# FraPria/proovread

Hardware: AMD Instinct MI355X
Metric: corrected long-read Mbases/sec per node (higher is better)
Workload: dtype int32

## Files before the change

### proovread_amd/csrc/seed.cpp

```cpp
#include <algorithm>
#include <atomic>
#include <cstdlib>
#include <cstring>
#include <string>
#include <thread>
#include <utility>
#include <vector>

#include <sys/mman.h>

#include "../../include/prgpu.h"
#include "err.h"
#include "seed_core.h"
#include "seed_dev.h"

namespace seedc = prgpu::seedc;

namespace {

constexpr int KI = 12;
constexpr uint32_t NK = 1u << (2 * KI);
constexpr uint8_t SEP = 5;
constexpr int KX = 28;
constexpr uint64_t KX_MASK = (1ull << (2 * KX)) - 1;

template <class T>
struct BigAlloc {
    using value_type = T;
    static constexpr size_t kHuge = (size_t)32 << 20;
    BigAlloc() = default;
    template <class U>
    BigAlloc(const BigAlloc<U> &) {}
    T *allocate(size_t n) {
        const size_t bytes = n * sizeof(T);
        if (bytes >= kHuge) {
// ... 620 lines not shown
        uint64_t v = 0;
        for (int k = 0; k < 16; ++k) {
            const int64_t x = (int64_t)w * 16 + k;
            v |= (uint64_t)(x < V.n_text ? V.text[x] : SEP) << (4 * k);
        }
        text4[w] = v;
    }
    return text4;
}

extern "C" int pr_seed_map_device_caps(const pr_seed_index *h, const pr_seed_opts *o, const uint8_t *sr_seq,
                                       const int64_t *sr_off, int n_sr, int n_threads, pr_seed_tasks *out,
                                       int32_t *status) {
    if (!h || !o || !out || !status || n_sr < 0 || (n_sr && (!sr_seq || !sr_off)))
        return pr_set_error(PR_ERR_ARG, "null arg");
    if (o->min_seed_len < KI) return pr_set_error(PR_ERR_UNSUPPORTED, "min seed length below the 12-mer index");
    out->n = 0;
    out->t = nullptr;
    seedc::IndexView V = view_of(h->I);
    int qmax = 1;
    for (int i = 0; i < n_sr; ++i) qmax = std::max<int>(qmax, (int)(sr_off[i + 1] - sr_off[i]));
    const std::vector<uint64_t> text4 = pack_text4(V);
    V.text4 = text4.data();
    seedc::Caps caps = seedc::device_caps(qmax);
    caps.hi = V.ksplit != nullptr;
    caps.lazy = seedc::lazy_occ(*o) ? 1 : 0;
    const int64_t bytes = seedc::scratch_bytes(caps);
    int nt = n_threads > 0 ? n_threads : (int)std::thread::hardware_concurrency();
    nt = nt < 1 ? 1 : (nt > 64 ? 64 : nt);
    std::vector<ReadOut> res(n_sr);
    std::atomic<int> next{0};
    const char *fe = getenv("PRGPU_SCRATCH_FILL");
    const uint64_t fill = fe ? 0x0101010101010101ull * (uint64_t)(strtoul(fe, nullptr, 0) & 0xFF) : 0;
    auto work = [&]() {
        std::vector<uint64_t> slab((size_t)(bytes / 8 + 1), fill);
        seedc::Scratch S = seedc::carve(reinterpret_cast<uint8_t *>(slab.data()), caps);
        for (int k = 0; k < S.hsize; ++k) S.htab[k].key = -1;
        S.htab_clean = true;
        std::vector<pr_seed_task> buf((size_t)caps.out);
        std::vector<uint64_t> big;
        for (;;) {
            const int i = next.fetch_add(1);
            if (i >= n_sr) break;
            const int len = (int)(sr_off[i + 1] - sr_off[i]);
            int n = 0, err = 0;
            if (len > 0) err = seedc::map_read(V, *o, S, sr_seq + sr_off[i], len, i, buf.data(), caps.out, &n);
            seedc::Caps cg = caps;
            for (int pass = 3; pass <= 6 && err && !(err & (seedc::SC_OVER_LEN | seedc::SC_OVER_OUT)); ++pass) {
// ... 16 lines not shown
    for (auto &r : res) total += (int64_t)r.tasks.size();
    out->t = (pr_seed_task *)std::malloc(sizeof(pr_seed_task) * (size_t)(total > 0 ? total : 1));
    if (!out->t) return pr_set_error(PR_ERR_ARG, "out of host memory");
    int64_t k = 0;
    for (auto &r : res)
        for (auto &t : r.tasks) out->t[k++] = t;
    out->n = total;
    return 0;
}

extern "C" int pr_seed_map_device_pass1(const pr_seed_index *h, const pr_seed_opts *o, const uint8_t *sr_seq,
                                        const int64_t *sr_off, int n_sr, int budget, pr_seed_tasks *out, int32_t *status,
                                        int32_t *hits) {
    if (!h || !o || !out || !status || !hits || n_sr < 0 || budget < 0 || (n_sr && (!sr_seq || !sr_off)))
        return pr_set_error(PR_ERR_ARG, "null arg");
    if (o->min_seed_len < KI) return pr_set_error(PR_ERR_UNSUPPORTED, "min seed length below the 12-mer index");
    out->n = 0;
    out->t = nullptr;
    seedc::IndexView V = view_of(h->I);
    int qmax = 1;
    for (int i = 0; i < n_sr; ++i) qmax = std::max<int>(qmax, (int)(sr_off[i + 1] - sr_off[i]));
    const std::vector<uint64_t> text4 = pack_text4(V);
    V.text4 = text4.data();
    seedc::Caps caps = seedc::device_caps_small(std::min(qmax, seedc::device_caps(qmax).lmax));
    caps.hi = V.ksplit != nullptr;
    caps.lazy = seedc::lazy_occ(*o) ? 1 : 0;
    caps.budget = budget;
    std::vector<uint64_t> slab((size_t)(seedc::scratch_bytes(caps) / 8 + 1), 0);
    seedc::Scratch S = seedc::carve(reinterpret_cast<uint8_t *>(slab.data()), caps);
    for (int k = 0; k < S.hsize; ++k) S.htab[k].key = -1;
    S.htab_clean = true;
    std::vector<pr_seed_task> buf((size_t)caps.out), all;
    for (int i = 0; i < n_sr; ++i) {
        const int len = (int)(sr_off[i + 1] - sr_off[i]);
        int n = 0, err = 0;
        if (len > 0) err = seedc::map_read(V, *o, S, sr_seq + sr_off[i], len, i, buf.data(), caps.out, &n);
        status[i] = err;
        hits[i] = !caps.lazy || len <= 0 || (err & seedc::SC_OVER_LEN) ? 0 : (err & seedc::SC_OVER_HITS) ? S.lz[2] : S.lz[0];
        if (!err) all.insert(all.end(), buf.begin(), buf.begin() + n);
    }
    out->t = (pr_seed_task *)std::malloc(sizeof(pr_seed_task) * (all.empty() ? 1 : all.size()));
    if (!out->t) return pr_set_error(PR_ERR_ARG, "out of host memory");
    std::copy(all.begin(), all.end(), out->t);
    out->n = (int64_t)all.size();
    return 0;
}
```

### proovread_amd/csrc/seed_api.cpp

```cpp
#include <algorithm>
#include <climits>
#include <cstdio>
#include <cstdlib>
#include <cstring>
#include <vector>

#include "ctx.h"
#include "seed_index_dev.h"
#include "seed_plan.h"

static int seed_text4(pr_ctx *c, seedc::IndexView &v, hipStream_t s) {
    int rc = c->sd[SI_TEXT4].ensure((size_t)ix_pack4_words(v.n_text) * 8);
    if (rc) return rc;
    const int e = ix_pack4_launch(v.text, v.n_text, c->sd[SI_TEXT4].as<uint64_t>(), s);
    if (e) return set_error(PR_ERR_HIP, "text packing: %s", hipGetErrorString((hipError_t)e));
    v.text4 = c->sd[SI_TEXT4].as<uint64_t>();
    v.walk_nw = v.n_text > ((int64_t)64 << 24) ? 1 : 4;
    if (const char *w = getenv("PRGPU_SEED_WALK_NW"))
        v.walk_nw = atoi(w) == 1 ? 1 : 4;
    return 0;
}

static int upload_blk_fr(pr_ctx *c, seedc::IndexView &v, const int64_t *cstart, const int64_t *off, int n_lr,
                         int64_t l_pac, int64_t n_text, hipStream_t s) {
    const int64_t nb = (n_text >> seedc::CB_SHIFT) + 1;
    const int nc = 2 * n_lr;
    const int bs = 1 << seedc::CB_SHIFT;
    auto delta = [&](int ci) -> int64_t {
        if (ci < n_lr) return off[ci] - cstart[ci];
        const int rid = 2 * n_lr - 1 - ci;
        return 2 * l_pac - off[rid + 1] - cstart[ci];
    };
    std::vector<seedc::BlkFr> t((size_t)nb);
    int ci = 0;
    for (int64_t b = 0; b < nb; ++b) {
        const int64_t b0 = b << seedc::CB_SHIFT, b1 = b0 + bs;
        while (ci + 1 < nc && cstart[ci + 1] <= b0) ++ci;
        seedc::BlkFr &e = t[(size_t)b];
        e.c0 = ci;
        e.d0 = nc ? delta(ci) : 0;
        e.d1 = ci + 1 < nc ? delta(ci + 1) : 0;
        e.bnd = ci + 1 < nc && cstart[ci + 1] < b1 ? (int32_t)(cstart[ci + 1] - b0) : bs;
        e.bnd2 = ci + 2 < nc && cstart[ci + 2] < b1 ? (int32_t)(cstart[ci + 2] - b0) : bs;
    }
    int rc = c->sd[SI_BLKFR].ensure(t.size() * sizeof(seedc::BlkFr));
    if (rc) return rc;
    HIPCHK(hipMemcpyAsync(c->sd[SI_BLKFR].p, t.data(), t.size() * sizeof(seedc::BlkFr), hipMemcpyHostToDevice, s));
    HIPCHK(hipStreamSynchronize(s));
    v.blkfr = c->sd[SI_BLKFR].as<seedc::BlkFr>();
    return 0;
}

extern "C" int pr_seed_gpu_upload(pr_ctx *c, const pr_seed_index *h) {
    if (!c || !h) return set_error(PR_ERR_ARG, "null arg");
    HIPCHK(hipSetDevice(c->device));
    hipStream_t s = c->stream;
    const seedc::IndexView hv = seed_index_view(h);
    const SeedIndexSizes z = seed_index_sizes(h);
    DevBuf *D = c->sd;
    int rc;
    if ((rc = upload(D[SI_TEXT], hv.text, (size_t)z.text, s)) || (rc = upload(D[SI_CSTART], hv.cstart, (size_t)z.cstart, s)) ||
        (rc = upload(D[SI_CBLK], hv.cblk, (size_t)z.cblk, s)) || (rc = upload(D[SI_LROFF], hv.lr_off, (size_t)z.lr_off, s)) ||
        (rc = upload(D[SI_KOFF], hv.koff, (size_t)z.koff, s)) || (rc = upload(D[SI_KPOS], hv.kpos, (size_t)z.kpos, s)) ||
        (rc = upload(D[SI_KEXT], hv.kext, (size_t)z.kpos, s)) ||
        (z.ksplit && (rc = upload(D[SI_KSPLIT], hv.ksplit, (size_t)z.ksplit, s))))
        return rc;
    seedc::IndexView v = hv;
// ... 280 lines not shown
    int64_t waves;
    int64_t lanes2;
    int64_t chunk;
    int32_t budget;
    std::vector<int32_t> nout, st;
    std::vector<int64_t> pre;
    int64_t total = 0, bad = 0;
    int32_t bad_flags = 0;
};

void map_plan(SeedMap &M, const pr_seed_opts *o, const int64_t *sr_off) {
    pr_ctx *c = M.c;
    int qmax = 1;
    for (int i = 0; i < M.n_sr; ++i) qmax = std::max<int>(qmax, (int)(sr_off[i + 1] - sr_off[i]));
    M.qmax = qmax;
    seedc::Caps &caps = M.caps, &small = M.small;
    caps = seedc::device_caps(qmax);
    caps.hi = c->seed_view.ksplit != nullptr;
    caps.nopos = 1;
    small = seedc::device_caps_small(std::min(qmax, caps.lmax));
    small.hi = caps.hi;
    small.nopos = 1;
    small.lazy = seedc::lazy_occ(*o) ? 1 : 0;
    if (const char *sc = getenv("PRGPU_SEED_SMALL"))
        sscanf(sc, "%d,%d,%d,%d,%d", &small.hits, &small.iv, &small.mems, &small.seeds, &small.chains);
    M.budget = small.lazy ? seedp::PASS1_LAZY_BUDGET : 0;
    if (const char *bu = getenv("PRGPU_SEED_BUDGET")) M.budget = small.lazy ? std::max(0, atoi(bu)) : 0;
    SeedDev &K = M.K;
    K = SeedDev{};
    K.V = c->seed_view;
    K.O = *o;
    K.n_sr = M.n_sr;
    K.caps = small;
    K.stride = seedc::scratch_bytes(small);
    const char *wpc = getenv("PRGPU_SEED_WAVES_PER_CU");
    size_t fr = 0, tot = 0;
    (void)hipMemGetInfo(&fr, &tot);
    (void)hipGetLastError();
    const int per_cu = wpc ? atoi(wpc) : 16;
    const int64_t full = caps.hi ? 0 : (int64_t)c->n_cu * per_cu * 64 * K.stride;
    M.waves = seedp::pass1_waves(M.n_sr, c->n_cu, per_cu, getenv("PRGPU_SEED_BALANCE") != nullptr,
                                 seedp::pass1_budget((int64_t)fr, (int64_t)M.D[SB_SCRATCH].cap, full), K.stride);
    K.n_lanes = M.waves;
    M.lanes2 = (int64_t)c->n_cu * seed_slots_per_cu(c->seed_view.walk_nw);
    const char *ob = getenv("PRGPU_SEED_OUT_MB");
    M.chunk = seedp::out_chunk(ob ? std::max<int64_t>(1, atoll(ob)) << 20
// ... 356 lines not shown
```

### proovread_amd/csrc/seed_core.h

```cpp
#pragma once
#include <math.h>
#include <stdint.h>

#include "../../include/prgpu.h"

#if defined(__HIPCC__)
#define SC_HD __host__ __device__ inline
#else
#define SC_HD inline
#endif

#if defined(PR_SEED_STATS) && !defined(__HIP_DEVICE_COMPILE__)
extern unsigned long long pr_seed_stat_g[24];
#define SC_STAT(k, v) __atomic_fetch_add(&pr_seed_stat_g[k], (unsigned long long)(v), __ATOMIC_RELAXED)
#else
#define SC_STAT(k, v) ((void)0)
#endif

namespace prgpu {
namespace seedc {

constexpr int KI = 12;
constexpr uint32_t NK = 1u << (2 * KI);
constexpr int KX = 28;
// ... 135 lines not shown

SC_HD void text_to_fr(const IndexView &I, uint64_t p, int64_t &fr, int &rid) {
    const int c = contig_of(I, p);
    const int64_t o = (int64_t)p - I.cstart[c];
    if (c < I.n_lr) {
        rid = c;
        fr = I.lr_off[c] + o;
    } else {
        rid = 2 * I.n_lr - 1 - c;
        fr = I.l_pac + (I.l_pac - I.lr_off[rid + 1]) + o;
    }
}

SC_HD uint64_t pack_fr_blk(const IndexView &I, uint64_t p);

constexpr int FR_RID_BITS = 24;
SC_HD uint64_t pack_fr(const IndexView &I, uint64_t p) {
    int64_t fr;
    int rid;
    text_to_fr(I, p, fr, rid);
    return ((uint64_t)fr << FR_RID_BITS) | (uint64_t)rid;
}

SC_HD uint64_t pack_fr_blk(const IndexView &I, uint64_t p) {
    if (I.blkfr) {
        const BlkFr bt = I.blkfr[p >> CB_SHIFT];
        const int o = (int)(p & ((1u << CB_SHIFT) - 1u));
        int c = -1;
        int64_t d = 0;
        if (o < bt.bnd) c = bt.c0, d = bt.d0;
        else if (o < bt.bnd2) c = bt.c0 + 1, d = bt.d1;
        if (c >= 0) {
            const int rid = c < I.n_lr ? c : 2 * I.n_lr - 1 - c;
            return ((uint64_t)((int64_t)p + d) << FR_RID_BITS) | (uint64_t)rid;
        }
    }
    return pack_fr(I, p);
}

SC_HD uint64_t nib16c(const uint64_t *w4, uint64_t x) {
    const uint64_t w = x >> 4;
    const int sh = (int)(x & 15) * 4;
    const uint64_t lo = w4[w];
    return sh ? (lo >> sh) | (w4[w + 1] << (64 - sh)) : lo;
}

constexpr int LC_MAX = 6;
SC_HD constexpr int lc_off(int j) { return ((1 << (2 * j)) - 4) / 3; }
constexpr int LC_N = lc_off(LC_MAX + 1);

template <bool LZ> struct OccB;
SC_HD void materialize(const OccB<true> &occ, int a);
template <class OccT> struct occ_lazy { static constexpr bool value = false; };
template <> struct occ_lazy<OccB<true>> { static constexpr bool value = true; };

template <bool LZ>
struct OccB {
    const IndexView *I;
    const Scratch *S;
    const uint8_t *q;
// ... 200 lines not shown
#pragma unroll
    for (int k = 0; k < RK; ++k) top[k] = 0;
    int32_t n = 0;
    const int32_t code = a + KI <= len ? S.codes[a] : -1;
    if (code >= 0) {
        const uint64_t r0 = I.koff[code], r1 = I.koff[code + 1];
        const int64_t need = (int64_t)beg + (int64_t)(r1 - r0);
        if (need > S.lim_hits) {
            if (!(S.lz[1] & SC_OVER_HITS)) {
                int64_t all = 0;
                for (int x = 0; x + KI <= len; ++x) {
                    const int32_t cx = S.codes[x];
                    if (cx >= 0) all += (int64_t)(I.koff[cx + 1] - I.koff[cx]);
                }
                S.lz[2] = (int32_t)(all < (int64_t)1 << 30 ? all : (int64_t)1 << 30);
            }
            S.lz[1] |= SC_OVER_HITS;
        } else {
            n = (int32_t)(r1 - r0);
            const uint64_t qe = S.qext[a];
            const bool ranked = q[a] < 4;
            constexpr int MB = 4;
            for (uint64_t r = r0; r < r1; r += MB) {
                uint64_t pp[MB], ex[MB], fr[MB];
#pragma unroll
                for (int u = 0; u < MB; ++u) {
                    const bool ok = r + u < r1;
                    pp[u] = ok ? hit_pos(I, (uint32_t)code, r + u) : 0ull;
                    ex[u] = ok ? I.kext[r + u] : 0ull;
                }
#pragma unroll
                for (int u = 0; u < MB; ++u) fr[u] = r + u < r1 ? pack_fr_blk(I, pp[u]) : 0ull;
#pragma unroll
                for (int u = 0; u < MB; ++u) {
                    if (r + u >= r1) break;
                    const int ml = hit_ml(I, S, q, len, a, pp[u], ex[u], qe);
                    const int32_t k = beg + (int32_t)(r + u - r0);
                    const uint16_t v = (uint16_t)(ml < 65535 ? ml : 65535);
                    S.hml[k] = v;
                    S.hfr[k] = fr[u];
                    const int d = ml - KI;
#pragma unroll
                    for (int t = 0; t < HB; ++t) g[t] += d >= t ? 1u : 0u;
                    if (ranked) topk_insert(top, v);
                }
            }
        }
    }
    S.hoff[a] = beg;
    S.hend[a] = beg + n;
    S.lz[0] = beg + n;
    uint32_t *dst = S.ge + (int64_t)a * HB;
#pragma unroll
    for (int t = 0; t < HB; ++t) dst[t] = g[t];
    fill_rk_top(occ, S, q, len, a, top);
}

SC_HD int build_starts(const IndexView &I, Scratch &S, const uint8_t *q, int len) {
    if (len > S.lmax) return SC_OVER_LEN;
    for (int a = 0; a <= len; ++a) {
        S.codes[a] = -1;
        S.qext[a] = 0;
        S.hoff[a] = 0;
// ... 76 lines not shown
            const uint64_t r0 = I.koff[code], r1 = I.koff[code + 1];
            if ((int64_t)nh + (int64_t)(r1 - r0) > S.cap_hits) return SC_OVER_HITS;
            uint32_t *g = S.ge + (int64_t)a * HB;
            int32_t k = prev0;
            for (uint64_t r = r0; r < r1; ++r) {
                const uint64_t p = hit_pos(I, code, r);
                while (k < prev1 && get_hpos(S, k) + 1 < p) ++k;
                int ml;
                if (k < prev1 && get_hpos(S, k) + 1 == p && S.hml[k] > KI) {
                    ml = S.hml[k] - 1;
                } else {
                    const uint64_t ex = I.kext[r];
                    const uint64_t qe = S.qext[a];
                    const int le = (int)(ex >> 56), lq = (int)(qe >> 56);
                    const uint64_t x = (ex ^ qe) & KX_MASK;
                    int m = x ? ctz64(x) >> 1 : KX;
                    m = m < le ? m : le;
                    m = m < lq ? m : lq;
                    ml = KI + m;
                    if (m == KX)
                        while (a + ml < len && q[a + ml] < 4 && T[p + ml] == q[a + ml]) ++ml;
                }
                set_hpos(S, nh, p);
                S.hfr[nh] = pack_fr(I, p);
                S.hml[nh] = (uint16_t)(ml < 65535 ? ml : 65535);
                ++nh;
                ++g[ml - KI < HB - 1 ? ml - KI : HB - 1];
            }
            for (int t = HB - 2; t >= 0; --t) g[t] += g[t + 1];
        }
        prev0 = S.hoff[a];
        prev1 = nh;
    }
    for (int a = len - KI + 1 < 0 ? 0 : len - KI + 1; a <= len; ++a) S.hoff[a] = nh;
    const Occ occ{&I, &S, q, len, nullptr};
    for (int a = 0; a < len; ++a) fill_rk(occ, S, q, len, a);
    return 0;
}

SC_HD void iv_reverse(Iv *v, int n) {
    for (int i = 0, j = n - 1; i < j; ++i, --j) {
        const Iv t = v[i];
        v[i] = v[j];
        v[j] = t;
    }
}

// ... 323 lines not shown
        for (int j = 0; j < qn; ++j) {
            const int qj = q[qb + j];
            const int sc = (ti > 3 || qj > 3) ? -1 : (ti == qj ? O.a : -O.b);
            int h = hdiag + sc;
            const int e = E[j * stride];
            h = h > e ? h : e;
            h = h > f ? h : f;
            h = h > 0 ? h : 0;
            hdiag = H[j * stride];
            H[j * stride] = (T)h;
            best = best > h ? best : h;
            int en = e - O.e_del, eo = h - oe_del;
            en = en > eo ? en : eo;
            E[j * stride] = (T)(en > 0 ? en : 0);
            int fn = f - O.e_ins, fo = h - oe_ins;
            fn = fn > fo ? fn : fo;
            f = fn > 0 ? fn : 0;
        }
    }
    return best;
}

SC_HD void chain_flt(const pr_seed_opts &O, Scratch &S, int ncv, int *n_chains);
template <bool LZ = false>
SC_HD int chain_seq(const IndexView &I, const pr_seed_opts &O, Scratch &S, int nm, int *n_cv);

template <bool LZ = false>
SC_HD int map_chains(const IndexView &I, const pr_seed_opts &O, Scratch &S, const uint8_t *q, int len, int *n_chains,
                     unsigned long long *ticks = nullptr, const uint32_t *lcnt = nullptr) {
    *n_chains = 0;
    int err = 0;
#if defined(__HIP_DEVICE_COMPILE__)
    unsigned long long t_last = ticks ? __builtin_amdgcn_s_memrealtime() : 0ULL;
#endif
    const OccB<LZ> occ{&I, &S, q, len, lcnt};
    const int nm = collect_intv(occ, S, O, q, len, err, ticks);
    if (LZ) err |= S.lz[1];
    if (err) return err;
    SC_STAT(0, 1);
    SC_STAT(1, nm);
#if defined(__HIP_DEVICE_COMPILE__)
    if (ticks) t_last = __builtin_amdgcn_s_memrealtime();
#endif
    int ncv = 0;
    err = chain_seq<LZ>(I, O, S, nm, &ncv);
    if (LZ) err |= S.lz[1];
    if (err) return err;
    SC_TICK(3);
    SC_STAT(11, ncv);
    SC_STAT(12, (unsigned long long)ncv * ncv);
    chain_flt(O, S, ncv, n_chains);
    SC_TICK(4);
    return 0;
}

template <bool LZ>
SC_HD int chain_seq(const IndexView &I, const pr_seed_opts &O, Scratch &S, int nm, int *n_cv) {
    const bool clean_on_entry = S.htab_clean;
    int32_t ns = 0, ncv = 0, nrg = 0;
    if (!clean_on_entry)
        for (int k = 0; k < S.hsize; ++k) S.htab[k].key = -1;
    auto leave = [&](int rc) {
        if (clean_on_entry)
            for (int r = 0; r < nrg; ++r) S.htab[S.rg[r].pad[0]].key = -1;
        return rc;
    };
    for (int mi = 0; mi < nm; ++mi) {
        const Iv p = S.mems[mi];
        const int slen = p.end - p.start;
        if (LZ && !S.ready[p.start]) return leave(SC_OVER_HITS);
        const int32_t h0 = S.hoff[p.start], h1 = LZ ? S.hend[p.start] : S.hoff[p.start + 1];
        const int64_t np = p.occ;
        const int64_t step = np > O.max_occ ? np / O.max_occ : 1;
        int64_t fidx = 0, take = 0, count = 0;
        constexpr int CB = 8;
        int32_t k = h0;
        while (k < h1 && count < O.max_occ) {
            int32_t sel[CB];
            int nsel = 0;
            while (k < h1 && count < O.max_occ && nsel < CB) {
                uint16_t ml[8];
#pragma unroll
                for (int u = 0; u < 8; ++u) ml[u] = k + u < h1 ? S.hml[k + u] : (uint16_t)0;
                int u = 0;
                for (; u < 8 && k < h1 && count < O.max_occ && nsel < CB; ++u, ++k) {
                    if (ml[u] < slen) continue;
                    const bool use = fidx == take;
                    ++fidx;
                    if (!use) continue;
                    take += step;
                    ++count;
                    sel[nsel++] = k;
                }
            }
            int64_t rb[CB];
            int rd[CB], hsl[CB];
            int32_t key[CB];
#pragma unroll
            for (int u = 0; u < CB; ++u) {
                const uint64_t v = u < nsel ? S.hfr[sel[u]] : 0ull;
                rb[u] = (int64_t)(v >> FR_RID_BITS);
                rd[u] = (int)(v & ((1u << FR_RID_BITS) - 1u));
                key[u] = rd[u] * 2 + (rb[u] >= I.l_pac ? 1 : 0);
            }
#pragma unroll
            for (int u = 0; u < CB; ++u) hsl[u] = u < nsel ? range_slot(S, key[u]) : 0;
            bool opened = false;
            for (int u = 0; u < nsel; ++u) {
                SC_STAT(3, 1);
                Seed s;
                s.rbeg = rb[u];
                s.qbeg = (int16_t)p.start;
                s.len = (int16_t)slen;
                s.nx = -1;
                const int rid = rd[u];
                const int hs = opened ? range_slot(S, key[u]) : hsl[u];
                const RangeEnt e = S.htab[hs];
                const bool found = e.key == key[u];
                int at = -1;
                bool at_tail = false;
                if (found) {
                    RangeRec &R = S.rg[e.r];
                    SC_STAT(4, 1);
// ... 187 lines not shown
            while (j >= first && (out[j].rmax0 < t.rmax0 || (out[j].rmax0 == t.rmax0 && out[j].rank < t.rank))) --j;
            const pr_seed_task v = t;
            for (int m = no; m > j + 1; --m) out[m] = out[m - 1];
            out[j + 1] = v;
            ++no;
        }
        if (no == first) continue;
        r0 -= cs;
        r1 -= cs;
        for (int m = first; m < no; ++m) {
            out[m].rank = m - first;
            out[m].rmax0 = (int32_t)(r0 > 0 ? r0 : 0);
            out[m].rmax1 = (int32_t)(r1 < L ? r1 : L);
        }
        ++nkept;
    }
    *n_out = no;
    SC_STAT(14, nch);
    SC_STAT(15, no);
    SC_TICK(5);
    return 0;
}

template <bool LZ = false>
SC_HD int map_after_occ(const IndexView &I, const pr_seed_opts &O, Scratch &S, const uint8_t *q, int len, int sid,
                        pr_seed_task *out, int cap_out, int *n_out, unsigned long long *ticks = nullptr,
                        const uint32_t *lcnt = nullptr, int16_t *dp16 = nullptr) {
    *n_out = 0;
    int nch = 0;
    const int err = map_chains<LZ>(I, O, S, q, len, &nch, ticks, lcnt);
    if (err) return err;
    return map_output(I, O, S, q, len, sid, nch, out, cap_out, n_out, nullptr, ticks, dp16);
}
#undef SC_TICK

SC_HD int map_read(const IndexView &I, const pr_seed_opts &O, Scratch &S, const uint8_t *q, int len, int sid,
                   pr_seed_task *out, int cap_out, int *n_out) {
    *n_out = 0;
    if (S.hend) {
        const int err = build_starts(I, S, q, len);
        return err ? err : map_after_occ<true>(I, O, S, q, len, sid, out, cap_out, n_out);
    }
    const int err = build_occ(I, S, q, len);
    return err ? err : map_after_occ<false>(I, O, S, q, len, sid, out, cap_out, n_out);
}

SC_HD bool lazy_occ(const pr_seed_opts &O) { return O.min_seed_len >= 17; }

}
}

namespace prgpu {
namespace seedc {

struct Caps {
    int32_t lmax, hits, iv, mems, seeds, chains, out;
    int32_t hi;
    int32_t nopos;
    int32_t lazy;
    int32_t budget;
};
SC_HD int device_out_cap(int qmax) { return qmax > 192 ? 2 * ((qmax + 15) & ~15) : 384; }
SC_HD Caps device_caps(int qmax = 0) {
    Caps c{1024, 8192, 256, 1024, 8192, 4096, 384, 0};
    c.out = device_out_cap(qmax);
    if (qmax > 192) {
        const int l = (qmax + 15) & ~15;
        c.hits = c.hits > 48 * l ? c.hits : 48 * l;
        c.iv = c.iv > l / 2 ? c.iv : l / 2;
        c.mems = c.mems > 2 * l ? c.mems : 2 * l;
        c.seeds = c.seeds > 4 * l ? c.seeds : 4 * l;
        c.chains = c.chains > 2 * l ? c.chains : 2 * l;
    }
    return c;
}
SC_HD Caps device_caps_small(int lmax) {
    const int l = lmax < 16 ? 16 : (lmax + 15) & ~15;
    Caps c{l, 4096, 64, 512, 512, 384, device_out_cap(lmax), 0};
    if (l > 160) {
        c.hits = c.hits > 24 * l ? c.hits : 24 * l;
        c.iv = c.iv > l / 4 ? c.iv : l / 4;
        c.mems = c.mems > 2 * l ? c.mems : 2 * l;
        c.seeds = c.seeds > 2 * l ? c.seeds : 2 * l;
// ... 14 lines not shown
SC_HD int32_t range_table_size(int32_t chains) {
    int32_t h = 64;
    while (h < 2 * chains) h <<= 1;
    return h;
}

SC_HD int64_t scratch_bytes(const Caps &c) {
    int64_t b = 0;
    b += align8(4 * (int64_t)(c.lmax + 1));
    b += align8(8 * (int64_t)(c.lmax + 1));
    b += align8(4 * (int64_t)(c.lmax + 1));
    b += align8(4 * (int64_t)c.lmax * HB);
    if (!c.nopos) b += align8(4 * (int64_t)c.hits);
    b += align8(2 * (int64_t)c.hits);
    b += align8((int64_t)sizeof(Iv) * c.mems);
    b += 3 * align8((int64_t)sizeof(Iv) * c.iv);
    b += align8((int64_t)sizeof(Seed) * c.seeds);
    b += 2 * align8((int64_t)sizeof(Chain) * c.chains);
    b += 2 * align8(4 * (int64_t)c.chains);
    b += align8((int64_t)sizeof(RangeEnt) * range_table_size(c.chains));
    b = (b + 63) & ~(int64_t)63;
    b += align8((int64_t)sizeof(RangeRec) * c.chains);
    b += align8(2 * (int64_t)(c.lmax + 1) * RK);
    b += align8(8 * (int64_t)c.hits);
    if (c.hi && !c.nopos) b += align8((int64_t)c.hits);
    if (c.lazy) {
        b += align8(4 * (int64_t)(c.lmax + 1));
        b += align8((int64_t)(c.lmax + 1));
        b += align8(8 * (int64_t)(c.lmax / 16 + 4));
        b += align8(16);
    }
    return (b + 63) & ~(int64_t)63;
}

SC_HD Scratch carve(uint8_t *p, const Caps &c) {
    Scratch S{};
    auto take = [&p](int64_t bytes) {
        uint8_t *r = p;
        p += align8(bytes);
        return r;
    };
    S.lmax = c.lmax;
    S.hoff = (int32_t *)take(4 * (int64_t)(c.lmax + 1));
    S.qext = (uint64_t *)take(8 * (int64_t)(c.lmax + 1));
    S.codes = (int32_t *)take(4 * (int64_t)(c.lmax + 1));
    S.ge = (uint32_t *)take(4 * (int64_t)c.lmax * HB);
    S.hpos = c.nopos ? nullptr : (uint32_t *)take(4 * (int64_t)c.hits);
    S.hml = (uint16_t *)take(2 * (int64_t)c.hits);
    S.cap_hits = c.hits;
    S.lim_hits = c.lazy && c.budget > 0 && c.budget < c.hits ? c.budget : c.hits;
    S.mems = (Iv *)take((int64_t)sizeof(Iv) * c.mems);
    S.cap_mems = c.mems;
    S.m1 = (Iv *)take((int64_t)sizeof(Iv) * c.iv);
    S.curr = (Iv *)take((int64_t)sizeof(Iv) * c.iv);
    S.prev = (Iv *)take((int64_t)sizeof(Iv) * c.iv);
    S.cap_iv = c.iv;
    S.seeds = (Seed *)take((int64_t)sizeof(Seed) * c.seeds);
    S.cap_seeds = c.seeds;
    S.cv = (Chain *)take((int64_t)sizeof(Chain) * c.chains);
    S.ch = (Chain *)take((int64_t)sizeof(Chain) * c.chains);
    S.cnx = (int32_t *)take(4 * (int64_t)c.chains);
    S.kept = (int32_t *)take(4 * (int64_t)c.chains);
    S.hsize = range_table_size(c.chains);
    S.htab = (RangeEnt *)take((int64_t)sizeof(RangeEnt) * S.hsize);
    p = (uint8_t *)(((uintptr_t)p + 63) & ~(uintptr_t)63);
    S.rg = (RangeRec *)take((int64_t)sizeof(RangeRec) * c.chains);
    S.cap_chains = c.chains;
    S.rmax = (uint16_t *)take(2 * (int64_t)(c.lmax + 1) * RK);
    S.hfr = (uint64_t *)take(8 * (int64_t)c.hits);
    S.hhi = c.hi && !c.nopos ? (uint8_t *)take((int64_t)c.hits) : nullptr;
    if (c.lazy) {
        S.hend = (int32_t *)take(4 * (int64_t)(c.lmax + 1));
        S.ready = (uint8_t *)take((int64_t)(c.lmax + 1));
        S.q4w = (uint64_t *)take(8 * (int64_t)(c.lmax / 16 + 4));
        S.lz = (int32_t *)take(16);
    }
    return S;
}

}
}
```

### proovread_amd/csrc/seed_kernels.hip

```cpp
#include <hip/hip_runtime.h>

#include <rocprim/device/device_radix_sort.hpp>

#include "seed_core.h"
#include "seed_dev.h"

namespace prgpu {

#ifndef SEED_WAVES_DEF
#define SEED_WAVES_DEF 4
#endif
#ifndef SEED_LMAX_DEF
#define SEED_LMAX_DEF 1024
#endif
constexpr int SEED_WAVES = SEED_WAVES_DEF;
constexpr int SEED_LMAX = SEED_LMAX_DEF;
#ifndef SEED_MINB
#define SEED_MINB 4
#endif
#ifndef SEED_WAVE_MINB
#define SEED_WAVE_MINB SEED_MINB
#endif
#ifndef OCC_U
#define OCC_U 2
// ... 677 lines not shown
                pt[0] += tm - t0;
                atomicMax(&D.prof[17], tm - t0);
            }
            if (len > 0 && !err) {
                const seedc::Occ occ{&D.V, &S, q, len, lcnt};
                nm = seedc::collect_intv(occ, S, D.O, q, len, err, D.prof ? pl : nullptr);
            }
            if (D.prof) atomicMax(&D.prof[18], wall_clock64() - tm);
        }
        err = __shfl(err, 0, 64);
        nm = __shfl(nm, 0, 64);
        if (len > 0 && !err) {
            const unsigned long long tc = D.prof && lane == 0 ? wall_clock64() : 0ULL;
            __threadfence_block();
            int ncv = chain_wave(D.V, D.O, S, nm, lane, ho);
            unsigned long long tf = D.prof && lane == 0 ? wall_clock64() : 0ULL;
            if (lane == 0 && D.prof) atomicAdd(&D.prof[14 + (ncv == -1 ? 1 : 0)], tf - tc);
            if (ncv == -2) {
                ncv = 0;
                err = seedc::SC_OVER_CHAINS;
            }
            if (lane == 0 && ncv == -1) {
                ncv = 0;
                err = seedc::chain_seq(D.V, D.O, S, nm, &ncv);
                if (D.prof) {
                    const unsigned long long t_ = wall_clock64();
                    atomicAdd(&D.prof[13], 1ULL);
                    atomicAdd(&D.prof[15], t_ - tf);
                    tf = t_;
                }
            }
            err = __shfl(err, 0, 64);
            ncv = __shfl(ncv, 0, 64);
            __threadfence_block();
            wave_sync_lds();
            bool flt = err != 0 || chain_flt_wave(D.O, S, ncv, lane, &nch);
            if (lane == 0) {
                if (!flt) seedc::chain_flt(D.O, S, ncv, &nch);
                if (D.prof) {
                    const unsigned long long t_ = wall_clock64();
                    pl[3] += t_ - tc;
                    atomicAdd(&D.prof[16], t_ - tf);
                }
                if (!err && seedc::seed_flt_min_score(D.O, len) >= 0 && 3 * S.cap_seeds <= 2 * S.cap_hits &&
                    2 * 201 * 64 * 2 <= 4 * S.lmax * seedc::HB)
                    nlist = seedc::flt_seed_list(S, nch, (int32_t *)S.hfr + S.cap_seeds, S.cap_seeds);
            }
// ... 87 lines not shown
        int my_err = 0, my_hits = 0;
        const int nb = (int)(nlim - b0 < batch ? nlim - b0 : batch);
        for (int rd = 0; rd < nb; ++rd) {
            const int i = D.rlist ? D.rlist[b0 + rd] : b0 + rd;
            const int64_t o = D.sr_off[i];
            const int len = (int)(D.sr_off[i + 1] - o);
            seedc::Scratch S = seedc::carve(base + (int64_t)rd * D.stride, D.caps);
            int err = 0, nh = 0;
            if (len > S.lmax || len > SEED_LMAX - 1) err = seedc::SC_OVER_LEN;
            if (len > 0 && !err)
                err = build_occ_wave<4>(D.V, S, D.sr_seq + o, len, ho, lane, q4_lds[wv], lcnt, &nh, D.prof ? ot : nullptr,
                                     LZ);
            if (lane == rd) my_err = err, my_hits = nh;
        }
        const unsigned long long t1 = D.prof ? wall_clock64() : 0ULL;
        if (lane < nb) {
            const int i = D.rlist ? D.rlist[b0 + lane] : b0 + lane;
            const int64_t o = D.sr_off[i];
            const int len = (int)(D.sr_off[i + 1] - o);
            seedc::Scratch S = seedc::carve(base + (int64_t)lane * D.stride, D.caps);
            S.htab_clean = HTAB_REUSE;
            int n = 0, err = my_err;
            if (len > 0 && !err)
                err = seedc::map_after_occ<LZ>(D.V, D.O, S, D.sr_seq + o, len, i, D.out + (int64_t)(i - D.out0) * D.caps.out,
                                           D.caps.out, &n, D.prof ? lt : nullptr, lcnt,
                                           D.dp ? D.dp + slot * (2 * 201 * 64) + lane : nullptr);
            D.n_out[i] = (my_err & seedc::SC_OVER_HITS) ? -my_hits
                         : (LZ && (err & seedc::SC_OVER_HITS)) ? -S.lz[2]
                                                                        : (err ? 0 : n);
            D.status[i] = err;
        }
        if (D.prof && lane == 0) {
            pt[0] += t1 - t0;
            pt[1] += wall_clock64() - t1;
        }
        __threadfence_block();
    }
}

__global__ void __launch_bounds__(256) seed_cost_kernel(seedc::IndexView V, const uint8_t *sr_seq, const int64_t *sr_off,
                                                        int64_t r0, int64_t n, uint32_t *key, int32_t *val) {
    for (int64_t k = (int64_t)blockIdx.x * blockDim.x + threadIdx.x; k < n; k += (int64_t)gridDim.x * blockDim.x) {
        const int64_t i = r0 + k;
        const int64_t o = sr_off[i];
        const int len = (int)(sr_off[i + 1] - o);
        uint32_t code = 0u, cost = 0u;
        int valid = 0;
        for (int p = 0; p < len; ++p) {
            const uint32_t c = sr_seq[o + p];
// ... 69 lines not shown
            A.d_off[k] = d_off[k0 + k];
            A.len[k] = len[k0 + k];
            lmax = std::max(lmax, A.len[k]);
        }
        const int64_t tiles = std::max<int64_t>(1, std::min<int64_t>(256, (lmax + GATHER_TILE - 1) / GATHER_TILE));
        hipLaunchKernelGGL(sr_gather_kernel, dim3((unsigned)tiles, (unsigned)m), dim3(256), 0, (hipStream_t)stream, src, dst, A);
        const hipError_t e = hipGetLastError();
        if (e != hipSuccess) return (int)e;
    }
    return 0;
}

int seed_slots_per_cu(int walk_nw) {
    int nb = 0;
    const hipError_t e = walk_nw == 1 ? hipOccupancyMaxActiveBlocksPerMultiprocessor(&nb, seed_wave_kernel<1>, 64 * SEED_WAVES, 0)
                                      : hipOccupancyMaxActiveBlocksPerMultiprocessor(&nb, seed_wave_kernel<4>, 64 * SEED_WAVES, 0);
    if (e != hipSuccess || nb < 1)
        nb = 2;
    return nb * SEED_WAVES;
}

int seed_launch(const SeedDev &D, void *stream) {
    if (D.n_list <= 0) return 0;
    const int64_t blocks = (D.n_lanes + SEED_WAVES - 1) / SEED_WAVES;
    if (D.V.walk_nw == 1)
        hipLaunchKernelGGL(seed_wave_kernel<1>, dim3((unsigned)blocks), dim3(64 * SEED_WAVES), 0, (hipStream_t)stream, D);
    else
        hipLaunchKernelGGL(seed_wave_kernel<4>, dim3((unsigned)blocks), dim3(64 * SEED_WAVES), 0, (hipStream_t)stream, D);
    return (int)hipGetLastError();
}

int seed_batch_launch(const SeedDev &D, void *stream) {
    if (D.n_sr <= 0) return 0;
    if (D.caps.lazy && (D.batch < 1 || D.batch > 64)) return (int)hipErrorInvalidValue;
    const int64_t blocks = (D.n_lanes + SEED_WAVES - 1) / SEED_WAVES;
    if (D.caps.lazy)
        hipLaunchKernelGGL(seed_batch_kernel<true>, dim3((unsigned)blocks), dim3(64 * SEED_WAVES), 0, (hipStream_t)stream, D);
    else
        hipLaunchKernelGGL(seed_batch_kernel<false>, dim3((unsigned)blocks), dim3(64 * SEED_WAVES), 0, (hipStream_t)stream, D);
    return (int)hipGetLastError();
}

__global__ void seed_compact_kernel(const pr_seed_task *slots, const int32_t *n_out, const int64_t *pre, int64_t n_sr,
                                    int cap, pr_seed_task *out) {
    const int64_t i = ((int64_t)blockIdx.x * blockDim.x + threadIdx.x) >> 6;
    const int lane = threadIdx.x & 63;
    if (i >= n_sr) return;
    const int n = n_out[i];
    constexpr int TW = (int)(sizeof(pr_seed_task) / 4);
    const uint32_t *src = reinterpret_cast<const uint32_t *>(slots + i * cap);
    uint32_t *dst = reinterpret_cast<uint32_t *>(out + pre[i]);
    for (int k = lane; k < n * TW; k += 64) dst[k] = src[k];
}

int seed_compact_launch(const pr_seed_task *slots, const int32_t *n_out, const int64_t *pre, int64_t n_sr, int cap,
                        pr_seed_task *out, void *stream) {
    if (n_sr <= 0) return 0;
// ... 8 lines not shown
```

Before: 232.4.

## Drop stored per-hit forward-read array in lazy path; recompute from positions at chaining

In the lazy-occurrence batch path, per-hit packed read/offset values (hfr) are no longer stored in scratch. Chaining recomputes them from stored hit positions via the block table, batched four at a time to overlap loads. The aim is less scratch memory and fewer global writes per hit, which may allow better occupancy or cache use. The cost is extra block-table lookups at chain time. Block-table construction moves into a shared header, and launch-time checks reject inconsistent cap combinations.

```diff
diff --git a/proovread_amd/csrc/seed.cpp b/proovread_amd/csrc/seed.cpp
--- a/proovread_amd/csrc/seed.cpp
+++ b/proovread_amd/csrc/seed.cpp
@@ -11,6 +11,7 @@
 
 #include "../../include/prgpu.h"
 #include "err.h"
+#include "seed_blkfr.h"
 #include "seed_core.h"
 #include "seed_dev.h"
 
@@ -677,8 +678,11 @@
     for (int i = 0; i < n_sr; ++i) qmax = std::max<int>(qmax, (int)(sr_off[i + 1] - sr_off[i]));
     const std::vector<uint64_t> text4 = pack_text4(V);
     V.text4 = text4.data();
+    const std::vector<seedc::BlkFr> blkfr = seedc::build_blk_fr(V.cstart, V.lr_off, V.n_lr, V.l_pac, V.n_text);
+    V.blkfr = blkfr.data();
     seedc::Caps caps = seedc::device_caps(qmax);
     caps.hi = V.ksplit != nullptr;
+    caps.nofr = 1;
     caps.lazy = seedc::lazy_occ(*o) ? 1 : 0;
     const int64_t bytes = seedc::scratch_bytes(caps);
     int nt = n_threads > 0 ? n_threads : (int)std::thread::hardware_concurrency();
@@ -741,8 +745,11 @@
     for (int i = 0; i < n_sr; ++i) qmax = std::max<int>(qmax, (int)(sr_off[i + 1] - sr_off[i]));
     const std::vector<uint64_t> text4 = pack_text4(V);
     V.text4 = text4.data();
+    const std::vector<seedc::BlkFr> blkfr = seedc::build_blk_fr(V.cstart, V.lr_off, V.n_lr, V.l_pac, V.n_text);
+    V.blkfr = blkfr.data();
     seedc::Caps caps = seedc::device_caps_small(std::min(qmax, seedc::device_caps(qmax).lmax));
     caps.hi = V.ksplit != nullptr;
+    caps.nofr = 1;
     caps.lazy = seedc::lazy_occ(*o) ? 1 : 0;
     caps.budget = budget;
     std::vector<uint64_t> slab((size_t)(seedc::scratch_bytes(caps) / 8 + 1), 0);
diff --git a/proovread_amd/csrc/seed_api.cpp b/proovread_amd/csrc/seed_api.cpp
--- a/proovread_amd/csrc/seed_api.cpp
+++ b/proovread_amd/csrc/seed_api.cpp
@@ -6,6 +6,7 @@
 #include <vector>
 
 #include "ctx.h"
+#include "seed_blkfr.h"
 #include "seed_index_dev.h"
 #include "seed_plan.h"
 
@@ -23,26 +24,7 @@
 
 static int upload_blk_fr(pr_ctx *c, seedc::IndexView &v, const int64_t *cstart, const int64_t *off, int n_lr,
                          int64_t l_pac, int64_t n_text, hipStream_t s) {
-    const int64_t nb = (n_text >> seedc::CB_SHIFT) + 1;
-    const int nc = 2 * n_lr;
-    const int bs = 1 << seedc::CB_SHIFT;
-    auto delta = [&](int ci) -> int64_t {
-        if (ci < n_lr) return off[ci] - cstart[ci];
-        const int rid = 2 * n_lr - 1 - ci;
-        return 2 * l_pac - off[rid + 1] - cstart[ci];
-    };
-    std::vector<seedc::BlkFr> t((size_t)nb);
-    int ci = 0;
-    for (int64_t b = 0; b < nb; ++b) {
-        const int64_t b0 = b << seedc::CB_SHIFT, b1 = b0 + bs;
-        while (ci + 1 < nc && cstart[ci + 1] <= b0) ++ci;
-        seedc::BlkFr &e = t[(size_t)b];
-        e.c0 = ci;
-        e.d0 = nc ? delta(ci) : 0;
-        e.d1 = ci + 1 < nc ? delta(ci + 1) : 0;
-        e.bnd = ci + 1 < nc && cstart[ci + 1] < b1 ? (int32_t)(cstart[ci + 1] - b0) : bs;
-        e.bnd2 = ci + 2 < nc && cstart[ci + 2] < b1 ? (int32_t)(cstart[ci + 2] - b0) : bs;
-    }
+    const std::vector<seedc::BlkFr> t = seedc::build_blk_fr(cstart, off, n_lr, l_pac, n_text);
     int rc = c->sd[SI_BLKFR].ensure(t.size() * sizeof(seedc::BlkFr));
     if (rc) return rc;
     HIPCHK(hipMemcpyAsync(c->sd[SI_BLKFR].p, t.data(), t.size() * sizeof(seedc::BlkFr), hipMemcpyHostToDevice, s));
@@ -369,6 +351,8 @@
     small.hi = caps.hi;
     small.nopos = 1;
     small.lazy = seedc::lazy_occ(*o) ? 1 : 0;
+    small.nopos = small.lazy ? 0 : 1;
+    small.nofr = small.lazy;
     if (const char *sc = getenv("PRGPU_SEED_SMALL"))
         sscanf(sc, "%d,%d,%d,%d,%d", &small.hits, &small.iv, &small.mems, &small.seeds, &small.chains);
     M.budget = small.lazy ? seedp::PASS1_LAZY_BUDGET : 0;
diff --git a/proovread_amd/csrc/seed_blkfr.h b/proovread_amd/csrc/seed_blkfr.h
--- /dev/null
+++ b/proovread_amd/csrc/seed_blkfr.h
@@ -0,0 +1,37 @@
+#pragma once
+#include <stdint.h>
+
+#include <vector>
+
+#include "seed_core.h"
+
+namespace prgpu {
+namespace seedc {
+
+inline std::vector<BlkFr> build_blk_fr(const int64_t *cstart, const int64_t *off, int n_lr, int64_t l_pac, int64_t n_text) {
+    const int64_t nb = (n_text >> CB_SHIFT) + 1;
+    const int nc = 2 * n_lr;
+    const int bs = 1 << CB_SHIFT;
+    auto delta = [&](int ci) -> int64_t {
+        if (ci < n_lr) return off[ci] - cstart[ci];
+        const int rid = 2 * n_lr - 1 - ci;
+        return 2 * l_pac - off[rid + 1] - cstart[ci];
+    };
+    std::vector<BlkFr> t((size_t)nb);
+    int ci = 0;
+    for (int64_t b = 0; b < nb; ++b) {
+        const int64_t b0 = b << CB_SHIFT, b1 = b0 + bs;
+        while (ci + 1 < nc && cstart[ci + 1] <= b0) ++ci;
+        BlkFr &e = t[(size_t)b];
+        e.c0 = ci;
+        e.d0 = nc ? delta(ci) : 0;
+        e.d1 = ci + 1 < nc ? delta(ci + 1) : 0;
+        e.bnd = ci + 1 < nc && cstart[ci + 1] < b1 ? (int32_t)(cstart[ci + 1] - b0) : bs;
+        e.bnd2 = ci + 2 < nc && cstart[ci + 2] < b1 ? (int32_t)(cstart[ci + 2] - b0) : bs;
+        e.pad = 0;
+    }
+    return t;
+}
+
+}
+}
diff --git a/proovread_amd/csrc/seed_core.h b/proovread_amd/csrc/seed_core.h
--- a/proovread_amd/csrc/seed_core.h
+++ b/proovread_amd/csrc/seed_core.h
@@ -181,20 +181,54 @@
     return ((uint64_t)fr << FR_RID_BITS) | (uint64_t)rid;
 }
 
+SC_HD uint64_t pack_fr_ent(const IndexView &I, const BlkFr &bt, uint64_t p) {
+    const int o = (int)(p & ((1u << CB_SHIFT) - 1u));
+    int c = -1;
+    int64_t d = 0;
+    if (o < bt.bnd) c = bt.c0, d = bt.d0;
+    else if (o < bt.bnd2) c = bt.c0 + 1, d = bt.d1;
+    if (c >= 0) {
+        const int rid = c < I.n_lr ? c : 2 * I.n_lr - 1 - c;
+        return ((uint64_t)((int64_t)p + d) << FR_RID_BITS) | (uint64_t)rid;
+    }
+    return pack_fr(I, p);
+}
 SC_HD uint64_t pack_fr_blk(const IndexView &I, uint64_t p) {
-    if (I.blkfr) {
-        const BlkFr bt = I.blkfr[p >> CB_SHIFT];
-        const int o = (int)(p & ((1u << CB_SHIFT) - 1u));
-        int c = -1;
-        int64_t d = 0;
-        if (o < bt.bnd) c = bt.c0, d = bt.d0;
-        else if (o < bt.bnd2) c = bt.c0 + 1, d = bt.d1;
-        if (c >= 0) {
-            const int rid = c < I.n_lr ? c : 2 * I.n_lr - 1 - c;
-            return ((uint64_t)((int64_t)p + d) << FR_RID_BITS) | (uint64_t)rid;
-        }
-    }
-    return pack_fr(I, p);
+    return I.blkfr ? pack_fr_ent(I, I.blkfr[p >> CB_SHIFT], p) : pack_fr(I, p);
+}
+
+SC_HD uint64_t hit_fr(const IndexView &I, const Scratch &S, int64_t k) {
+    return S.hfr ? S.hfr[k] : pack_fr_blk(I, get_hpos(S, k));
+}
+enum { FR_ANY = 0, FR_STORED = 1, FR_LOOKUP = 2 };
+template <int FRM, int N>
+SC_HD void hit_fr_batch(const IndexView &I, const Scratch &S, const int32_t (&sel)[N], const uint64_t (&p)[N], int nsel,
+                        uint64_t (&v)[N]) {
+    if (FRM == FR_STORED || (FRM == FR_ANY && S.hfr)) {
+#pragma unroll
+        for (int u = 0; u < N; ++u) v[u] = u < nsel ? S.hfr[sel[u]] : 0ull;
+        return;
+    }
+    constexpr int FRG = 4;
+    static_assert(N % FRG == 0, "a batch is whole block-table groups");
+#pragma unroll
+    for (int g = 0; g < N; g += FRG) {
+        if (g >= nsel) {
+#pragma unroll
+            for (int u = 0; u < FRG; ++u) v[g + u] = 0ull;
+            continue;
+        }
+        if (I.blkfr) {
+            BlkFr bt[FRG];
+#pragma unroll
+            for (int u = 0; u < FRG; ++u) bt[u] = I.blkfr[(g + u < nsel ? p[g + u] : 0ull) >> CB_SHIFT];
+#pragma unroll
+            for (int u = 0; u < FRG; ++u) v[g + u] = g + u < nsel ? pack_fr_ent(I, bt[u], p[g + u]) : 0ull;
+        } else {
+#pragma unroll
+            for (int u = 0; u < FRG; ++u) v[g + u] = g + u < nsel ? pack_fr(I, p[g + u]) : 0ull;
+        }
+    }
 }
 
 SC_HD uint64_t nib16c(const uint64_t *w4, uint64_t x) {
@@ -441,15 +475,13 @@
             const bool ranked = q[a] < 4;
             constexpr int MB = 4;
             for (uint64_t r = r0; r < r1; r += MB) {
-                uint64_t pp[MB], ex[MB], fr[MB];
+                uint64_t pp[MB], ex[MB];
 #pragma unroll
                 for (int u = 0; u < MB; ++u) {
                     const bool ok = r + u < r1;
                     pp[u] = ok ? hit_pos(I, (uint32_t)code, r + u) : 0ull;
                     ex[u] = ok ? I.kext[r + u] : 0ull;
                 }
-#pragma unroll
-                for (int u = 0; u < MB; ++u) fr[u] = r + u < r1 ? pack_fr_blk(I, pp[u]) : 0ull;
 #pragma unroll
                 for (int u = 0; u < MB; ++u) {
                     if (r + u >= r1) break;
@@ -457,7 +489,8 @@
                     const int32_t k = beg + (int32_t)(r + u - r0);
                     const uint16_t v = (uint16_t)(ml < 65535 ? ml : 65535);
                     S.hml[k] = v;
-                    S.hfr[k] = fr[u];
+                    set_hpos(S, k, pp[u]);
+                    if (S.hfr) S.hfr[k] = pack_fr_blk(I, pp[u]);
                     const int d = ml - KI;
 #pragma unroll
                     for (int t = 0; t < HB; ++t) g[t] += d >= t ? 1u : 0u;
@@ -580,7 +613,7 @@
                         while (a + ml < len && q[a + ml] < 4 && T[p + ml] == q[a + ml]) ++ml;
                 }
                 set_hpos(S, nh, p);
-                S.hfr[nh] = pack_fr(I, p);
+                if (S.hfr) S.hfr[nh] = pack_fr(I, p);
                 S.hml[nh] = (uint16_t)(ml < 65535 ? ml : 65535);
                 ++nh;
                 ++g[ml - KI < HB - 1 ? ml - KI : HB - 1];
@@ -950,10 +983,10 @@
 }
 
 SC_HD void chain_flt(const pr_seed_opts &O, Scratch &S, int ncv, int *n_chains);
-template <bool LZ = false>
+template <bool LZ = false, int FRM = FR_ANY>
 SC_HD int chain_seq(const IndexView &I, const pr_seed_opts &O, Scratch &S, int nm, int *n_cv);
 
-template <bool LZ = false>
+template <bool LZ = false, int FRM = FR_ANY>
 SC_HD int map_chains(const IndexView &I, const pr_seed_opts &O, Scratch &S, const uint8_t *q, int len, int *n_chains,
                      unsigned long long *ticks = nullptr, const uint32_t *lcnt = nullptr) {
     *n_chains = 0;
@@ -971,7 +1004,7 @@
     if (ticks) t_last = __builtin_amdgcn_s_memrealtime();
 #endif
     int ncv = 0;
-    err = chain_seq<LZ>(I, O, S, nm, &ncv);
+    err = chain_seq<LZ, FRM>(I, O, S, nm, &ncv);
     if (LZ) err |= S.lz[1];
     if (err) return err;
     SC_TICK(3);
@@ -982,7 +1015,7 @@
     return 0;
 }
 
-template <bool LZ>
+template <bool LZ, int FRM>
 SC_HD int chain_seq(const IndexView &I, const pr_seed_opts &O, Scratch &S, int nm, int *n_cv) {
     const bool clean_on_entry = S.htab_clean;
     int32_t ns = 0, ncv = 0, nrg = 0;
@@ -1005,11 +1038,18 @@
         int32_t k = h0;
         while (k < h1 && count < O.max_occ) {
             int32_t sel[CB];
+            uint64_t selp[CB];
             int nsel = 0;
+            const bool lookup = FRM == FR_LOOKUP || (FRM == FR_ANY && !S.hfr);
             while (k < h1 && count < O.max_occ && nsel < CB) {
                 uint16_t ml[8];
+                uint32_t pl[8] = {0u, 0u, 0u, 0u, 0u, 0u, 0u, 0u};
 #pragma unroll
                 for (int u = 0; u < 8; ++u) ml[u] = k + u < h1 ? S.hml[k + u] : (uint16_t)0;
+                if (lookup) {
+#pragma unroll
+                    for (int u = 0; u < 8; ++u) pl[u] = k + u < h1 ? S.hpos[k + u] : 0u;
+                }
                 int u = 0;
                 for (; u < 8 && k < h1 && count < O.max_occ && nsel < CB; ++u, ++k) {
                     if (ml[u] < slen) continue;
@@ -1018,15 +1058,18 @@
                     if (!use) continue;
                     take += step;
                     ++count;
+                    if (lookup) selp[nsel] = (uint64_t)pl[u] | (S.hhi ? (uint64_t)S.hhi[k] << 32 : 0ull);
                     sel[nsel++] = k;
                 }
             }
             int64_t rb[CB];
             int rd[CB], hsl[CB];
             int32_t key[CB];
+            uint64_t fr[CB];
+            hit_fr_batch<FRM>(I, S, sel, selp, nsel, fr);
 #pragma unroll
             for (int u = 0; u < CB; ++u) {
-                const uint64_t v = u < nsel ? S.hfr[sel[u]] : 0ull;
+                const uint64_t v = fr[u];
                 rb[u] = (int64_t)(v >> FR_RID_BITS);
                 rd[u] = (int)(v & ((1u << FR_RID_BITS) - 1u));
                 key[u] = rd[u] * 2 + (rb[u] >= I.l_pac ? 1 : 0);
@@ -1260,13 +1303,13 @@
     return 0;
 }
 
-template <bool LZ = false>
+template <bool LZ = false, int FRM = FR_ANY>
 SC_HD int map_after_occ(const IndexView &I, const pr_seed_opts &O, Scratch &S, const uint8_t *q, int len, int sid,
                         pr_seed_task *out, int cap_out, int *n_out, unsigned long long *ticks = nullptr,
                         const uint32_t *lcnt = nullptr, int16_t *dp16 = nullptr) {
     *n_out = 0;
     int nch = 0;
-    const int err = map_chains<LZ>(I, O, S, q, len, &nch, ticks, lcnt);
+    const int err = map_chains<LZ, FRM>(I, O, S, q, len, &nch, ticks, lcnt);
     if (err) return err;
     return map_output(I, O, S, q, len, sid, nch, out, cap_out, n_out, nullptr, ticks, dp16);
 }
@@ -1297,6 +1340,7 @@
     int32_t nopos;
     int32_t lazy;
     int32_t budget;
+    int32_t nofr;
 };
 SC_HD int device_out_cap(int qmax) { return qmax > 192 ? 2 * ((qmax + 15) & ~15) : 384; }
 SC_HD Caps device_caps(int qmax = 0) {
@@ -1357,7 +1401,7 @@
     b = (b + 63) & ~(int64_t)63;
     b += align8((int64_t)sizeof(RangeRec) * c.chains);
     b += align8(2 * (int64_t)(c.lmax + 1) * RK);
-    b += align8(8 * (int64_t)c.hits);
+    if (!c.nofr) b += align8(8 * (int64_t)c.hits);
     if (c.hi && !c.nopos) b += align8((int64_t)c.hits);
     if (c.lazy) {
         b += align8(4 * (int64_t)(c.lmax + 1));
@@ -1402,7 +1446,7 @@
     S.rg = (RangeRec *)take((int64_t)sizeof(RangeRec) * c.chains);
     S.cap_chains = c.chains;
     S.rmax = (uint16_t *)take(2 * (int64_t)(c.lmax + 1) * RK);
-    S.hfr = (uint64_t *)take(8 * (int64_t)c.hits);
+    S.hfr = c.nofr ? nullptr : (uint64_t *)take(8 * (int64_t)c.hits);
     S.hhi = c.hi && !c.nopos ? (uint8_t *)take((int64_t)c.hits) : nullptr;
     if (c.lazy) {
         S.hend = (int32_t *)take(4 * (int64_t)(c.lmax + 1));
diff --git a/proovread_amd/csrc/seed_kernels.hip b/proovread_amd/csrc/seed_kernels.hip
--- a/proovread_amd/csrc/seed_kernels.hip
+++ b/proovread_amd/csrc/seed_kernels.hip
@@ -723,7 +723,7 @@
             }
             if (lane == 0 && ncv == -1) {
                 ncv = 0;
-                err = seedc::chain_seq(D.V, D.O, S, nm, &ncv);
+                err = seedc::chain_seq<false, seedc::FR_STORED>(D.V, D.O, S, nm, &ncv);
                 if (D.prof) {
                     const unsigned long long t_ = wall_clock64();
                     atomicAdd(&D.prof[13], 1ULL);
@@ -857,9 +857,9 @@
             S.htab_clean = HTAB_REUSE;
             int n = 0, err = my_err;
             if (len > 0 && !err)
-                err = seedc::map_after_occ<LZ>(D.V, D.O, S, D.sr_seq + o, len, i, D.out + (int64_t)(i - D.out0) * D.caps.out,
-                                           D.caps.out, &n, D.prof ? lt : nullptr, lcnt,
-                                           D.dp ? D.dp + slot * (2 * 201 * 64) + lane : nullptr);
+                err = seedc::map_after_occ<LZ, LZ ? seedc::FR_LOOKUP : seedc::FR_STORED>(
+                    D.V, D.O, S, D.sr_seq + o, len, i, D.out + (int64_t)(i - D.out0) * D.caps.out, D.caps.out, &n,
+                    D.prof ? lt : nullptr, lcnt, D.dp ? D.dp + slot * (2 * 201 * 64) + lane : nullptr);
             D.n_out[i] = (my_err & seedc::SC_OVER_HITS) ? -my_hits
                          : (LZ && (err & seedc::SC_OVER_HITS)) ? -S.lz[2]
                                                                         : (err ? 0 : n);
@@ -975,6 +975,7 @@
 
 int seed_launch(const SeedDev &D, void *stream) {
     if (D.n_list <= 0) return 0;
+    if (D.caps.nofr) return (int)hipErrorInvalidValue;
     const int64_t blocks = (D.n_lanes + SEED_WAVES - 1) / SEED_WAVES;
     if (D.V.walk_nw == 1)
         hipLaunchKernelGGL(seed_wave_kernel<1>, dim3((unsigned)blocks), dim3(64 * SEED_WAVES), 0, (hipStream_t)stream, D);
@@ -986,6 +987,7 @@
 int seed_batch_launch(const SeedDev &D, void *stream) {
     if (D.n_sr <= 0) return 0;
     if (D.caps.lazy && (D.batch < 1 || D.batch > 64)) return (int)hipErrorInvalidValue;
+    if (D.caps.lazy ? (!D.caps.nofr || D.caps.nopos) : D.caps.nofr) return (int)hipErrorInvalidValue;
     const int64_t blocks = (D.n_lanes + SEED_WAVES - 1) / SEED_WAVES;
     if (D.caps.lazy)
         hipLaunchKernelGGL(seed_batch_kernel<true>, dim3((unsigned)blocks), dim3(64 * SEED_WAVES), 0, (hipStream_t)stream, D);
```

After: 229.8. 1.1% lower.
